# Yash-10/beta-sgp

Measured on AMD Instinct MI355X. Metric: SGP iterations/sec (fp64) on batched 256x256 images, higher is better.
Workload: dtype f64; 1 GPU; C3: 1024 independent 256x256 stamps per GPU, 25x25 PSF, linear A, beta-SGP (beta=1.05), proj_type=1, MAXIT=100, stop_criterion=1; images_per_gpu=1024, images_total=1024, maxit=100, parallelism=1 independent shards, one process per GPU (no collective on the data path), ls_spec=2, streams=1, team=1, proj_cache=1, gn_compact=1, storage=f64, persistent=1, stop_criterion=1

## Files before the change

### beta-sgp_amd/_bsgp.py

```python
import ctypes
import os
import threading

import numpy as np

try:
    import torch
except ImportError:
    torch = None

_HERE = os.path.dirname(os.path.abspath(__file__))
LIB_PATH = os.environ.get("BSGP_LIB", os.path.join(_HERE, "libbsgp.so"))

BSGP_CONV_CIRCULAR = 0
BSGP_CONV_LINEAR_FILL = 1
BSGP_VARIANT_KL = 0
BSGP_VARIANT_BETA = 1
BSGP_STORAGE_F64 = 0
BSGP_STORAGE_F32 = 1
ABI_VERSION = 3
BSGP_ERR_ARG = -1
BSGP_ERR_HIP = -2
BSGP_ERR_UNSUPPORTED = -3
BSGP_ERR_PSF = -4
# ... 595 lines not shown
        raise ValueError(f"storage must be 'f64' or 'f32', not {storage!r}")
    return STORAGE[storage]


_libc = ctypes.CDLL(None)
_libc.memcmp.restype = ctypes.c_int
_libc.memcmp.argtypes = [ctypes.c_void_p, ctypes.c_void_p, ctypes.c_size_t]


def _same_psf(plan, psf):
    ref = plan._psf_host
    return ref.shape == psf.shape and (
        psf.nbytes == 0 or _libc.memcmp(ref.ctypes.data, psf.ctypes.data, psf.nbytes) == 0)


_PLAN_KNOBS = ("BSGP_PERWAVE_MIN_WG", "BSGP_PERWAVE_TW", "BSGP_COOP_ELEMS", "BSGP_LS_PREDICT")


def _plan_key(H, W, psf, conv_mode, storage):
    psf = np.ascontiguousarray(psf, dtype="<f8")
    flat = psf.reshape(-1)
    sample = flat[::max(1, flat.size // 4096)].tobytes()
    return psf, (H, W, psf.shape, hash(sample), conv_mode, storage_code(storage),
                 torch.cuda.current_device(), tuple(os.environ.get(k) for k in _PLAN_KNOBS))


def _new_plan(H, W, psf, key):
    p = Plan(H, W, psf, key[4], key[6], storage=key[5], psf_checked=True)
    p._psf_host = psf.copy()
    return p

# ... 139 lines not shown
```

### beta-sgp_amd/csrc/bsgp_device.hpp

```cpp
#pragma once

#include <hip/hip_runtime.h>
#include <stdint.h>

#include <type_traits>

#include "bsgp_fft.hpp"
#include "bsgp_lanesplit.hpp"
#include "bsgp_math.hpp"
#include "bsgp_reduce.hpp"

namespace bsgp {

constexpr int kTeamFlags = 64;
constexpr int kPartBufs = 3;
constexpr unsigned long long kPartEmpty = 0xFFF75EE0FFF75EE0ull;
constexpr unsigned int kPartEmptyWord = 0xFFF75EE0u;
constexpr int kSharedBytes = 512;

constexpr int kPhaseSlots = 40;
#ifdef BSGP_PHASE_PROF
static __device__ unsigned long long g_phase[kPhaseSlots];
#define PH_T(v) const unsigned long long v = __builtin_amdgcn_s_memtime()
#define PH_ADD(slot, t0)                                                                 \
// ... 48 lines not shown
struct SGeo {
  static constexpr int H = H_, W = W_, P = P_, Q = Q_;
  static constexpr int Qh = Q_ / 2 + 1;
  static constexpr int nfw = kWaves, nfc = kWaves, coop = 0;
  static constexpr int maxlen = P_ > Q_ ? P_ : Q_;
  static constexpr int lpad = (maxlen + 1 > 2 * Qh ? maxlen + 1 : 2 * Qh) | 1;
  static constexpr int sld = H_ + (H_ & 1);
  static constexpr int tw2 = 0, twmix = -1;
  static constexpr int lds_fft_bytes = nfw * 2 * lpad * (int)sizeof(cd);
  static constexpr int lds_tw_p =
      lds_fft_bytes + kWaves * kMaxRed * (int)sizeof(double) + kSharedBytes;
  static constexpr int lds_tw_q = P_ == Q_ ? lds_tw_p : lds_tw_p + P_ * (int)sizeof(cd);
  static constexpr int lds_bytes = lds_tw_q + Q_ * (int)sizeof(cd);
  static constexpr SPlan<P_, lds_tw_p> fp{};
  static constexpr SPlan<Q_, lds_tw_q> fq{};
  const cd* tfA;
  const cd* tfAT;
  size_t tf_stride;
};
template <class GT>
struct IsStaticGeo : std::false_type {};
template <int H_, int W_, int P_, int Q_>
struct IsStaticGeo<SGeo<H_, W_, P_, Q_>> : std::true_type {};
using SGeo256 = SGeo<256, 256, 270, 270>;
static_assert(SGeo256::Qh == 136 && SGeo256::sld == 256 && SGeo256::lpad == 273, "geometry");

template <bool COMP = true, int N, int OFF, class Sync>
__device__ __forceinline__ cd* fft_any(cd* a, cd* b, const SPlan<N, OFF>&, bool inv, int lane,
                                       int nlanes, Sync sync) {
  extern __shared__ __attribute__((aligned(16))) char bsgp_dyn_lds[];
  const cd* t = reinterpret_cast<const cd*>(bsgp_dyn_lds + OFF);
  return fft_run_static<N, COMP>(a, b, t, inv, lane, nlanes, sync);
}

__device__ __forceinline__ void copy_tw(const FftPlan& f) {
  if (f.lds_tw < 0) return;
  extern __shared__ __attribute__((aligned(16))) char bsgp_dyn_lds[];
  cd* d = reinterpret_cast<cd*>(bsgp_dyn_lds + f.lds_tw);
  for (int i = threadIdx.x; i < f.n; i += kBlock) d[i] = f.tw[i];
}
// ... 1284 lines not shown
      A[u] = ldp<NT>(col);
      const cd bk = ldp<NT>(col + (two ? 1 : 0));
      B[u] = two ? bk : cmk(0.0, 0.0);
    }
#pragma unroll
    for (int u = 0; u < kGCH; ++u) {
      const int k = k0 + 64 * u;
      if (k < G.Qh) {
        a[k] = cmk(A[u].x - B[u].y, A[u].y + B[u].x);
        if (k > 0 && G.Q - k >= G.Qh) a[G.Q - k] = cmk(A[u].x + B[u].y, B[u].x - A[u].y);
      }
    }
  }
}

typedef __attribute__((address_space(3))) void lds_void_t;
typedef __attribute__((address_space(1))) void gbl_void_t;
template <unsigned POL = 0, class GT = Geo>
__device__ __forceinline__ void stage_pair(const GT& G, const cd* spec, int ld, int r, bool two,
                                           cd* F, int lane) {
  constexpr int kAux = (POL & kNtSR) ? 2 : 0;
  for (int k0 = 0; k0 < G.Qh; k0 += 32) {
    const int k = k0 + (lane >> 1);
    if (k < G.Qh) {
      const cd* col = spec + (size_t)k * ld + r + (two ? (lane & 1) : 0);
      __builtin_amdgcn_global_load_lds((gbl_void_t*)col, (lds_void_t*)(F + 2 * k0), 16, 0, kAux);
    }
  }
}
template <class GT = Geo>
// ... 133 lines not shown
        }
        in2[j] = cmk(va, vb);
      }
      wave_sync();
      cd* Y = fft_any(in2, Z, G.fq, false, lane, 64, WaveSync());
      for (int k = lane; k < G.Qh; k += 64) {
        cd ak, bk;
        r2c_split(Y, G.Q, k, &ak, &bk);
        store_pair(spec + (size_t)k * G.sld + r, two, pair_ok, ak, bk);
      }
      wave_sync();
    }
  }
}

template <int JCH = kJCH, bool COMP = true, unsigned POL = 0, class LD, class CP, class GT = Geo>
__device__ __forceinline__ void row_inv_fwd2(const GT& G, const Part& D, const cd* src, cd* dst,
                                             cd* lds, LD&& ld, CP&& cp) {
  using V = decltype(ld(0, 0));
  const int w = threadIdx.x >> 6, lane = threadIdx.x & 63;
  const bool pair_ok = (G.sld & 1) == 0;
  if (w < G.nfw) {
    cd* a = lds + w * 2 * G.lpad;
    cd* b = a + G.lpad;
    for (int r = 2 * (D.gw0 + w); r < G.H; r += 2 * D.gws) {
      const bool two = row_two(G, r, G.H);
      gather_pair<POL>(G, src, G.sld, r, two, a, lane);
      V v0[JCH], v1[JCH];
      load_rows<JCH>(ld, r, two, 0, lane, G.W, v0, v1);
      wave_sync();
      cd* Z = fft_any<COMP>(a, b, G.fq, true, lane, 64, WaveSync());
      cd* in2 = (Z == a) ? b : a;
      for (int j0 = 0; j0 < G.Q; j0 += 64 * JCH) {
        if (j0 > 0 && j0 < G.W) load_rows<JCH>(ld, r, two, j0, lane, G.W, v0, v1);
#pragma unroll
        for (int u = 0; u < JCH; ++u) {
          const int j = j0 + 64 * u + lane;
          if (j < G.Q) {
            double va = 0.0, vb = 0.0;
            if (j < G.W) {
              const cd z = Z[j];
              va = cp(r, j, z.x, v0[u]);
              if (two) vb = cp(r + 1, j, z.y, v1[u]);
            }
            in2[j] = cmk(va, vb);
          }
        }
      }
      wave_sync();
      cd* Y = fft_any<COMP>(in2, Z, G.fq, false, lane, 64, WaveSync());
      for (int k = lane; k < G.Qh; k += 64) {
        cd ak, bk;
        r2c_split(Y, G.Q, k, &ak, &bk);
        store_pair<POL>(dst + (size_t)k * G.sld + r, two, pair_ok, ak, bk);
      }
      wave_sync();
    }
  }
}

template <bool COOP = false, unsigned POL = 0, class GT = Geo>
__device__ __forceinline__ void col_conv(const GT& G, const Part& D, cd* spec, const cd* tf,
                                         cd* lds) {
  constexpr bool NT = (POL & kNtSC) != 0;
  if constexpr (COOP) {
    coop_col_conv(G, D, spec, tf, lds);
    return;
  }
  const int w = threadIdx.x >> 6, lane = threadIdx.x & 63;
// ... 353 lines not shown
```

### beta-sgp_amd/csrc/bsgp_internal.hpp

```cpp
#pragma once

#include <hip/hip_runtime.h>

#include <vector>

#include "../../include/bsgp.h"
#include "bsgp_device.hpp"

namespace bsgp {

struct ImgState {
  int par, Xones, stop, iter, epoch;
  int bar_base;
  int64_t E_p, E_ls, ls_passes, status, ls_series;
  int64_t proj_passes, proj_list;
  double sc, flux, bks_scalar, lo, hi, Dcoeff, tol, t0;
  double fv, alpha, tau, lr, init_lr, beta, lam_p, gd, lam;
  double lam_ratio, kappa;
  double konst;
  int g32;
  int par_tf;
  int par_spec;
  double gfill;
  double Valpha[32];
// ... 29 lines not shown
  unsigned int* tctr;
  int* tfail;
  double* plist;
  size_t plist_stride;
  int lcap;
  int list_lds;
  PwProg pw;
  int storage;
  size_t spec_off;
  int ls_cap;
  unsigned spin_limit;
  int fold_setup;
  int ls_predict;
  cd* spec2;
  size_t spec2_stride;
};

hipError_t launch_setup(const SolveArgs& a, size_t lds, hipStream_t s);
hipError_t launch_iteration(const SolveArgs& a, int K, size_t lds, hipStream_t s,
                            hipEvent_t* ev = nullptr);
hipError_t launch_track(const SolveArgs& a, int it, hipStream_t s);
hipError_t launch_build_tf(const Geo& g, const double* kc, cd* spec, cd* tf, double scale,
                           int conj, size_t lds, hipStream_t s);
hipError_t launch_build_tfs(const Geo& g, int n, const double* kc, size_t kc_stride, cd* spec,
                            size_t spec_stride, cd* tf, size_t tf_stride, double scale, int conj,
                            size_t lds, hipStream_t s);
hipError_t launch_place_psfs(const Geo& g, int n, const double* psfs, int kh, int kw, int circ,
                             double* kc, double* sums, hipStream_t s);
hipError_t launch_apply_op(const Geo& g, int B, int transpose, const double* x, double* out,
                           cd* specws, size_t spec_stride, int grid, size_t lds, hipStream_t s);
// ... 5 lines not shown
                             int max_projs, double* x, double* info, hipStream_t s);
hipError_t launch_beta_div(int n, const double* y, const double* x, double beta, double* out,
                           hipStream_t s);
hipError_t launch_beta_div_deriv(int64_t n, const double* y, const double* x, double beta,
                                 double* out, hipStream_t s);
hipError_t launch_grad_parts(int64_t n, const double* den, const double* gn, double beta,
                             double* pow1, double* w, hipStream_t s);
hipError_t set_solver_lds_limit(size_t bytes);
hipError_t team_resident_per_cu(bool coop, int storage, size_t lds, int* per_cu);
hipError_t phase_prof(unsigned long long* out, int n, int reset);
hipError_t launch_persist(const SolveArgs& a, int K, size_t lds, hipStream_t s, unsigned* queue,
                          unsigned* done, int grid);
hipError_t persist_resident_per_cu(const SolveArgs& a, int K, size_t lds, int* per_cu);
bool persist_static_geo(const SolveArgs& a, int K);
bool persist_speculates(const SolveArgs& a);
hipError_t persist_phase_prof(unsigned long long* out, int n, int reset);
void persist_kernels_all(std::vector<const void*>& f);

static_assert(sizeof(bsgp_state_header) <= BSGP_STATE_HEADER_BYTES, "state header overflows");

struct StateLayout {
  size_t bytes, discr, crit, times, flags, x, g, xtf, pw, gn, bkg;
};
inline size_t state_pad16(size_t v) { return (v + 15) / 16 * 16; }
inline StateLayout state_layout(size_t N, int storage, bool bmap, int hist_cap) {
  const size_t vb = storage == BSGP_STORAGE_F32 ? 4 : 8;
  StateLayout L{};
  size_t o = BSGP_STATE_HEADER_BYTES;
  auto take = [&](size_t n) {
    const size_t at = o;
// ... 68 lines not shown
```

### beta-sgp_amd/csrc/bsgp_kernels.hpp

```cpp
#pragma once

#include <hip/hip_runtime.h>

#include <type_traits>
#include <vector>

#include "bsgp_device.hpp"
#include "bsgp_internal.hpp"

namespace bsgp {


#ifndef BSGP_LS1_PRE
#define BSGP_LS1_PRE false
#endif
constexpr int kLs1Jch = 1;
#ifndef BSGP_COL_ATTR
#define BSGP_COL_ATTR
#endif
#ifndef BSGP_LS_ATTR
#define BSGP_LS_ATTR __attribute__((amdgpu_waves_per_eu(COOP ? 1 : ((K <= 2 && !ADAPT) ? 3 : 2))))
#endif
#ifndef BSGP_LS1_K2
#define BSGP_LS1_K2 0
#endif
#ifndef BSGP_PERSIST_LL
#define BSGP_PERSIST_LL 0
#endif
#ifndef BSGP_STREAM_NT
#define BSGP_STREAM_NT 0
#endif
#ifndef BSGP_STATIC_GEO
#define BSGP_STATIC_GEO 0
#endif
constexpr int kLsLanes = 32;
#ifndef BSGP_ACC_SERIES
#define BSGP_ACC_SERIES 0
#endif
constexpr int kLsAccJch = 1;
constexpr bool kLsAccPf = true;
#ifndef BSGP_LS1_PIPE
#define BSGP_LS1_PIPE false
// ... 543 lines not shown
    }
  }
}

template <bool COOP, class V>
__global__ void __launch_bounds__(kBlock) k_setup(SolveArgs A) {
  load_tw_lds(A.g);
  setup_phase<COOP, V>(A, team_img(A));
}

constexpr double kProjGuessW = 0.3;
constexpr double kProjW1 = 0.1;
constexpr double kProjW2 = 0.2;
constexpr int kProjWidePx = 16;

template <class V, bool LL, unsigned POL = 0>
__device__ __forceinline__ ProjOut cached_projection(const SolveArgs& A, int img, const Part& Pt, Team& tm,
                                     const Dir& D, const Bufs<V>& B, double* red, cd* lds,
                                     double lam_prev, double flux, int npair, bool odd, int N,
                                     int64_t& passes, int64_t& list_reads, double lam_ratio,
                                     double kappa, double& first_lam) {
  const V* xa = B.xa;
  const V* ga = B.ga;
  const int LS = tm.T * kBlock;
  const int gt = tm.m * kBlock + (int)threadIdx.x;
  double* ly = A.plist + (size_t)img * A.plist_stride;
  double* lX = ly + A.plist_stride / 2;
  const int lcap = A.lcap;
  const int nl = LL ? A.list_lds : 0;
  double* const qy = reinterpret_cast<double*>(lds);
  double* const qX = qy + (size_t)nl * kBlock;
  const int tl = (int)threadIdx.x;
  const bool hs = D.clip.has_sat;
  const double satv = D.clip.satv;
  bool have = false;
  double cL = 0.0, cU = 0.0, SA = 0.0, SB = 0.0, nsat = 0.0, nstr = 0.0;
  double Lk = -INFINITY, Uk = INFINITY;
  double xl0 = NAN, xs0 = 0.0, xl1 = NAN, xs1 = 0.0, lamN = NAN;
  bool first_miss = true;
  int calls = 0;
  int cnt = 0;

  auto note = [&](double lam, double S) {
    const double r = S - flux;
    if (r < 0 && lam > Lk) Lk = lam;
    if (r > 0 && lam < Uk) Uk = lam;
// ... 19 lines not shown
        t[k] += v;
        if (k == 0 && v > 0.0 && (!hs || v < satv)) t[NL + 5] += X;
      }
      if (split) {
        const double vL = D.pv(y, X, qL), vU = D.pv(y, X, qU);
        if (vU == 0.0) {
        } else if (hs && vL == satv) {
          t[NL + 2] += 1.0;
        } else if (vL > 0.0 && (!hs || vU < satv)) {
          t[NL] += y;
          t[NL + 1] += X;
        } else if (cnt < lcap) {
          if (cnt < nl) {
            qy[cnt * kBlock + tl] = y;
            qX[cnt * kBlock + tl] = X;
          } else {
            ly[(size_t)cnt * LS + gt] = y;
            lX[(size_t)cnt * LS + gt] = X;
          }
          ++cnt;
          t[NL + 3] += 1.0;
        } else {
          t[NL + 4] += 1.0;
        }
      }
    };
    stream2<kProjU>(
        Pt, npair,
        [&](int p) {
          struct Ld {
// ... 19 lines not shown
      SB = t[NL + 1];
      nsat = t[NL + 2];
      nstr = t[NL + 3];
    }
    ++passes;
    PH_ADD(NL == 3 ? 10 : 12, tp0);
    return t[NL + 5];
  };
  auto leval = [&](double lam) {
    PH_T(tl0);
    double t[1] = {0.0};
    int k = 0;
    if (nl > 0) {
      const int kl = cnt < nl ? cnt : nl;
      for (; k < kl; ++k) t[0] += D.pv(qy[k * kBlock + tl], qX[k * kBlock + tl], lam);
    }
    for (; k + 4 <= cnt; k += 4) {
      double yv[4], Xv[4];
#pragma unroll
      for (int u = 0; u < 4; ++u) {
        yv[u] = ly[(size_t)(k + u) * LS + gt];
        Xv[u] = lX[(size_t)(k + u) * LS + gt];
      }
#pragma unroll
      for (int u = 0; u < 4; ++u) t[0] += D.pv(yv[u], Xv[u], lam);
    }
    for (; k < cnt; ++k) t[0] += D.pv(ly[(size_t)k * LS + gt], lX[(size_t)k * LS + gt], lam);
    team_sum<1>(t, red, tm);
    PH_ADD(11, tl0);
    const double lin = SA + lam * SB;
// ... 51 lines not shown
        }
        first_miss = false;
        const double lams[1] = {lam};
        double Sv[1];
        (void)pass(std::integral_constant<int, 1>{}, lams, Sv, split, qL, qU);
        S = Sv[0];
      }
    }
    ++calls;
    note(lam, S);
    return S;
  };
  return project_df_fn(sumf, flux, 0.0, 1.0, 1e-11, 0, 0, A.prm.max_projs);
}

template <bool COOP, class V, bool LL = true, unsigned POL = 0, class GT = Geo>
__device__ __forceinline__ void dir_phase(const SolveArgs& A, int img) {
  constexpr bool kO16 = (POL & kNtO16) != 0, kO8 = (POL & kNtO8) != 0;
  BSGP_LDS_VIEWS_G(A, GT);
  ImgState& st = A.st[img];
  PH_T(tk0);
  Team tm = team_of<GT>(A, img, st);
  decltype(auto) G = geo_of<GT>(A);
  const Part Pt = make_part(tm, G.nfw, G.W);
  const bsgp_params& P = A.prm;
  const int N = G.H * G.W;
  const int npair = (N + 1) / 2;
  const bool odd = (N & 1) != 0;
  Bufs<V> B = slot_bufs<V>(A, img, st.par, st.par_tf);
  Dir D = make_dir(A, st);
  const double flux = st.flux;
// ... 216 lines not shown
      have2 = true;
      PH_ADD(34, tr0);
    }
  };
  bool spec_acc = false;
  bool spec_miss = false;
  if constexpr (kPredBuild) {
    if (pred == 1) {
      double ts[2] = {0.0, 0.0};
      const double bm1s = obj.beta - 1;
      V* const xs = B.xtf2;
      V* const ps = B.pw2;
      struct SpIn {
        double x0, g, bkv;
      };
      row_inv_fwd2<kLs1Jch, kLsComp, POL>(
          G, Pt, B.spec, B.spec2, lds,
          [&](int r, int j) {
            const int i = r * G.W + j;
            SpIn q;
            q.x0 = ldp<kO8>(B.xtf + i);
            q.g = g_raw<kO8>(g32, B.gns, i);
            q.bkv = opt_ld<kO8>(bmap, B.bks, i, bks_scalar);
            return q;
          },
          [&](int r, int j, double v, const SpIn& q) {
            const int i = r * G.W + j;
            const double g = gdec(q.g);
            const double xt = q.x0 + lam * v;
            const double den = xt + q.bkv;
            const double p = fpow(den, bm1s);
            ts[0] += obj.c1 * (den * p);
            ts[1] += (MODE == 4 ? (double)(obj.c2f * (float)g) : obj.c2 * g) * p;
            stp<kW>(xs + i, (V)xt);
            stp<kW>(ps + i, (V)p);
            return g * (p / den);
          });
      team_sum<2>(ts, red, tm);
      PH_ADD(37, tk0);
      ++passes;
      ++nls;
      const double f1 = obj.combine(konst, ts[0], ts[1], flux, (double)N);
      if (f1 <= fr + P.gamma * lam * gd || lam < 1e-12) {
        f_acc = f1;
        accepted = true;
        spec_acc = true;
      } else {
        spec_miss = true;
      }
    }
  }
  if (pred != 1 || spec_miss) {
// ... 521 lines not shown
__device__ __forceinline__ const SolveArgs& args_of(ArgRef r) {
  typedef const __attribute__((address_space(4))) SolveArgs* KP;
  const unsigned lo = (unsigned)__builtin_amdgcn_readfirstlane((int)r.lo);
  const unsigned hi = (unsigned)__builtin_amdgcn_readfirstlane((int)r.hi);
  const unsigned long long a = ((unsigned long long)hi << 32) | (unsigned long long)lo;
  KP p = (KP)a;
  asm volatile("" : "+s"(p));
  return *(const SolveArgs*)p;
}
template <bool COOP, class V>
__device__ __attribute__((noinline)) void persist_setup(ArgRef r, int img) {
  setup_phase<COOP, V>(args_of(r), __builtin_amdgcn_readfirstlane(img));
}
template <bool COOP, class V, unsigned POL, class GT = Geo>
__device__ __attribute__((noinline)) void persist_dir(ArgRef r, int img) {
  dir_phase<COOP, V, (BSGP_PERSIST_LL) != 0, POL, GT>(args_of(r),
                                                    __builtin_amdgcn_readfirstlane(img));
}
template <bool COOP, unsigned POL, class GT = Geo>
__device__ __attribute__((noinline)) void persist_col_a(ArgRef r, int img) {
  const SolveArgs& A = args_of(r);
  img = __builtin_amdgcn_readfirstlane(img);
  BSGP_LDS_VIEWS_G(A, GT);
  (void)red;
  Team tm{};
  tm.T = 1;
  const Bufs<double> Bd = slot_bufs<double>(A, img, 0);
  PH_T(tc0);
  decltype(auto) G = geo_of<GT>(A);
  col_conv<COOP, POL>(G, make_part(tm, COOP ? G.nfc : G.nfw, G.W), Bd.spec, tf_of(G, img, 0), lds);
  PH_ADD(3, tc0);
}
// ... 353 lines not shown
```

### beta-sgp_amd/csrc/bsgp_layout.hpp

```cpp
#pragma once

#include <algorithm>
#include <cerrno>
#include <cstddef>
#include <cstdlib>
#include <string>
#include <vector>

#include "../../include/bsgp.h"
#include "bsgp_fft.hpp"

namespace bsgp {

inline thread_local std::string g_err;

inline int fail(int code, const std::string& msg) {
  g_err = msg;
  return code;
}

inline size_t round_up(size_t v, size_t m) { return (v + m - 1) / m * m; }

inline long long env_knob(const char* name, long long def, long long lo, long long hi) {
  const char* e = getenv(name);
  if (!e || !*e) return def;
  char* end = nullptr;
  errno = 0;
  const long long v = strtoll(e, &end, 10);
  if (errno != 0 || end == e || *end != '\0' || v < lo || v > hi) return def;
  return v;
}

namespace layout {
constexpr int kWaves = 4, kMaxRed = 24, kSharedBytes = 512, kCoopBlock = 512, kCoopGroups = 4;
constexpr size_t kLdsPerCu = 160 * 1024;
}

struct PlanKnobs {
  int perwave_min_wg;
  int perwave_tw;
  int coop_elems;
  static PlanKnobs from_env() {
    return {(int)env_knob("BSGP_PERWAVE_MIN_WG", 2, 2, 4), (int)env_knob("BSGP_PERWAVE_TW", 1, 0, 1),
            (int)env_knob("BSGP_COOP_ELEMS", 8, 4, 8)};
  }
};

struct PlanLayout {
  int H, W, P, Q, Qh, sld, lpad, nfw, nfc, coop, tw2, twmix;
  FftPlan fp, fq;
// ... 47 lines not shown
    if (pmin < km) pmin = km;
    if (qmin < km) qmin = km;
    g.P = next_fast_len(pmin);
    g.Q = next_fast_len(qmin);
  }
  g.Qh = g.Q / 2 + 1;
  g.sld = H + ((H & 1) ? 1 : 0);
  g.fp.n = g.P;
  g.fq.n = g.Q;
  if (!plan_radices(g.P, g.fp.radix, &g.fp.ns) || !plan_radices(g.Q, g.fq.radix, &g.fq.ns))
    return fail(BSGP_ERR_UNSUPPORTED, "FFT length has too many factors");
  const int maxlen = g.P > g.Q ? g.P : g.Q;
  g.lpad = (maxlen + 1 > 2 * g.Qh ? maxlen + 1 : 2 * g.Qh) | 1;
  size_t red_bytes = (size_t)kWaves * kMaxRed * sizeof(double) + kSharedBytes;
  auto need = [&](int n) { return (size_t)n * 2 * g.lpad * sizeof(cd) + red_bytes; };
  auto budget_at = [](int wg) { return kLdsPerCu / wg - 256; };
  size_t budget = budget_at(4);
  g.wg_per_cu = 4;
  const size_t twb = (size_t)(g.P == g.Q ? g.P : g.P + g.Q) * sizeof(cd);
  const size_t tw_need = knobs.perwave_tw ? twb : 0;
  for (int wg = 3; wg >= 2 && wg >= knobs.perwave_min_wg; --wg)
    if (need(kWaves) > budget && need(kWaves) + tw_need <= budget_at(wg)) {
      budget = budget_at(wg);
      g.wg_per_cu = wg;
      break;
    }
  int nfw = kWaves;
  if (need(kWaves) > budget) {
    g.coop = 1;
    budget = budget_at(1);
    red_bytes = (size_t)(kCoopBlock / 64) * kMaxRed * sizeof(double) + kSharedBytes;
// ... 24 lines not shown
  if (g.coop) {
    place_coop_tables(&g);
  } else if (g.lds_bytes + twb <= budget) {
    g.fp.lds_tw = (int)g.lds_bytes;
    g.fq.lds_tw = g.P == g.Q ? g.fp.lds_tw : (int)(g.lds_bytes + (size_t)g.P * sizeof(cd));
    g.lds_bytes += twb;
  }
  g.vec_stride = round_up((size_t)H * W, 32);
  const size_t vbytes = storage == BSGP_STORAGE_F32 ? sizeof(float) : sizeof(double);
  g.spec_off = 2 * g.vec_stride + 7 * g.vec_stride * vbytes / sizeof(double);
  g.slot_stride = g.spec_off + round_up((size_t)g.sld * g.Qh * 2, 32) + 2 * g.vec_stride;
  *out = g;
  return BSGP_OK;
}

inline int check_plan_shape(int H, int W, int kh, int kw, int conv_mode, int storage) {
  if (storage != BSGP_STORAGE_F64 && storage != BSGP_STORAGE_F32)
    return fail(BSGP_ERR_ARG, "bad storage");
  if (H < 1 || W < 1 || kh < 1 || kw < 1) return fail(BSGP_ERR_ARG, "bad shape or psf");
  if (conv_mode != BSGP_CONV_CIRCULAR && conv_mode != BSGP_CONV_LINEAR_FILL)
    return fail(BSGP_ERR_ARG, "bad conv_mode");
  if (conv_mode == BSGP_CONV_CIRCULAR && (kh != H || kw != W))
    return fail(BSGP_ERR_ARG,
                "circular A (use_original_SGP_Afunction=True) needs psf.shape == gn.shape");
  return BSGP_OK;
}

struct PwBuild {
  std::vector<int> leaves, nodes_tmp, heights, roots;
  int rec(int start, int n, int* h) {
// ... 54 lines not shown
```

### beta-sgp_amd/csrc/bsgp_persist.hip

```cpp
#include <hip/hip_runtime.h>

#include <vector>

#ifndef BSGP_LS1_K2
#define BSGP_LS1_K2 1
#endif
#ifndef BSGP_STREAM_NT
#define BSGP_STREAM_NT 21
#endif
#ifndef BSGP_STATIC_GEO
#define BSGP_STATIC_GEO 1
#endif
#ifndef BSGP_PERSIST_LL
#define BSGP_PERSIST_LL 1
#endif
#include "bsgp_kernels.hpp"

namespace bsgp {

hipError_t launch_persist_f32(const SolveArgs& a, int K, size_t lds, hipStream_t s,
                              unsigned* queue, unsigned* done, int grid);
const void* persist_kernel_f32(int K, int mode, bool adapt, bool scalar_bkg);
void persist_kernels_f32(std::vector<const void*>& f);

hipError_t launch_persist(const SolveArgs& a, int K, size_t lds, hipStream_t s, unsigned* queue,
                          unsigned* done, int grid) {
  if (a.g.coop) return bsgp_c512_launch_persist(&a, K, lds, s, queue, done, grid);
  if (app_static_plan(a.g, a.storage))
    return bsgp_app_launch_persist(&a, K, lds, s, queue, done, grid);
// ... 3 lines not shown

bool persist_static_geo(const SolveArgs& a, int K) {
  if (a.g.coop || app_static_plan(a.g, a.storage) || a.storage != BSGP_STORAGE_F64) return false;
  bool adapt = false;
  const int mode = ls_mode(a, &adapt);
  return static_geo_kernel<double, (BSGP_STATIC_GEO != 0)>(false, K >= 2 ? 2 : K, mode, adapt) &&
         static_geo_plan(a);
}

bool persist_speculates(const SolveArgs& a) {
  if (a.g.coop || app_static_plan(a.g, a.storage) || a.storage != BSGP_STORAGE_F64) return false;
  bool adapt = false;
  const int mode = ls_mode(a, &adapt);
  return (BSGP_LS1_K2) != 0 && !adapt && (mode == 3 || mode == 4) && a.prm.ls_series != 0 &&
         a.T == 1 && a.ls_predict != 0;
}

hipError_t persist_resident_per_cu(const SolveArgs& a, int K, size_t lds, int* per_cu) {
  if (a.g.coop) return bsgp_c512_persist_resident(&a, K, lds, per_cu);
  if (app_static_plan(a.g, a.storage)) return bsgp_app_persist_resident(&a, K, lds, per_cu);
  bool adapt = false;
  const int mode = ls_mode(a, &adapt);
  const bool sb = !a.prm.bkg_is_map;
  const void* f = a.storage == BSGP_STORAGE_F32 ? persist_kernel_f32(K, mode, adapt, sb)
                                                : persist_kernel<double>(K, mode, adapt, sb);
  return hipOccupancyMaxActiveBlocksPerMultiprocessor(per_cu, f, kBlock, lds);
}

hipError_t persist_phase_prof_f32(unsigned long long* out, int n, int reset);
hipError_t persist_phase_prof(unsigned long long* out, int n, int reset) {
// ... 31 lines not shown
```

### beta-sgp_amd/csrc/bsgp_plan.hip

```cpp
#include <cmath>
#include <cstdio>
#include <memory>
#include <vector>

#include "bsgp_host.hpp"

using namespace bsgp;

static_assert(layout::kWaves == kWaves && layout::kMaxRed == kMaxRed &&
                  layout::kSharedBytes == kSharedBytes && layout::kCoopBlock == kCoopBlock &&
                  layout::kCoopGroups == kCoopGroups,
              "bsgp_layout.hpp restates the kernels' constants");

namespace {

std::vector<cd> twiddles(int n) {
  std::vector<cd> t(n);
  const long double pi = 3.141592653589793238462643383279502884L;
  for (int k = 0; k < n; ++k) {
    const long double a = -2.0L * pi * (long double)k / (long double)n;
    t[k] = cmk((double)cosl(a), (double)sinl(a));
  }
  return t;
}

void apply_layout(bsgp_plan p, const PlanLayout& l) {
// ... 284 lines not shown
```

### beta-sgp_amd/csrc/bsgp_solve.hip

```cpp
#include <algorithm>
#include <atomic>
#include <cmath>
#include <cstdio>
#include <cstring>
#include <string>
#include <vector>

#include "bsgp_host.hpp"

using namespace bsgp;

namespace {

int check_params(const bsgp_params* q) {
  if (!q) return fail(BSGP_ERR_ARG, "params is NULL");
  if (q->variant != BSGP_VARIANT_KL && q->variant != BSGP_VARIANT_BETA)
    return fail(BSGP_ERR_ARG, "bad variant");
  if (q->MAXIT < 1) return fail(BSGP_ERR_ARG, "MAXIT must be >= 1");
  if (q->M_alpha < 1 || q->M_alpha > 32) return fail(BSGP_ERR_ARG, "M_alpha must be in [1, 32]");
  if (q->M < 1 || q->M > 32) return fail(BSGP_ERR_ARG, "M must be in [1, 32]");
  if (q->ls_spec < 1 || q->ls_spec > 8) return fail(BSGP_ERR_ARG, "ls_spec must be in [1, 8]");
  if (q->init_recon < 0 || q->init_recon > 3) return fail(BSGP_ERR_ARG, "bad init_recon");
  if (q->proj_type != 0 && q->proj_type != 1) return fail(BSGP_ERR_ARG, "bad proj_type");
  if (q->scale_data < 0 || q->scale_data > 2) return fail(BSGP_ERR_ARG, "bad scale_data");
  if (q->flux_f32 && !(q->gn_f32 && q->scale_data != 2))
    return fail(BSGP_ERR_ARG, "flux_f32 needs gn_f32 with scale_data 0 or 1");
  return BSGP_OK;
}

struct SolveKnobs {
  unsigned spin_limit;
  int ls_predict;
  size_t list_lds;
  int static_geo;
  int fold_setup;
  static SolveKnobs from_env() {
    return {(unsigned)env_knob("BSGP_SPIN_LIMIT", 1ll << 26, 0, 0xffffffffll),
            (int)env_knob("BSGP_LS_PREDICT", 1, 0, 5),
            (size_t)env_knob("BSGP_LIST_LDS", 1 << 20, 0, 1 << 20),
            (int)env_knob("BSGP_STATIC_GEO", 1, 0, 1), (int)env_knob("BSGP_FOLD_SETUP", 1, 0, 1)};
  }
};

struct StaticGeoCall {
  bsgp_plan p;
  explicit StaticGeoCall(bsgp_plan q) : p(q) { p->last_static_geo = 0; }
  ~StaticGeoCall() { p->static_geo_next = -1; }
};

int proj_list_cap(const Geo& g, int T) {
  const long npair = ((long)g.H * g.W + 1) / 2;
  const int nb = plan_block(g);
  if (T == 1) return (int)(2 * ((npair + nb - 1) / nb));
  const long cp = (long)g.nfw * g.W;
  const long nch = (npair + cp - 1) / cp;
// ... 29 lines not shown
struct ResumeCtx {
  StateArgs sa;
  int T;
  int it0;
  bool uniform;
  int done_it;
  int beta0_given;
};

struct SolvePath {
  bool data_stop;
  bool track;
  bool persist;
  int K;
  int S;
};

int validate_solve(bsgp_plan p, int32_t B, const bsgp_params* prm, const bsgp_inputs* in,
                   const bsgp_outputs* out, bool resumed) {
  if (!p) return fail(BSGP_ERR_ARG, "plan is NULL");
  if (int rc = check_params(prm)) return rc;
  if (B < 1) return fail(BSGP_ERR_ARG, "B must be >= 1");
  if (!resumed) {
    if (!in || !in->gn || !in->bkg) return fail(BSGP_ERR_ARG, "inputs gn/bkg missing");
    if ((prm->init_recon == 1 || prm->scale_data == 2) && !in->x0)
      return fail(BSGP_ERR_ARG, "init_recon=1 and scale_data=2 need x0");
  }
  if (!out || !out->x || !out->iters || !out->discr) return fail(BSGP_ERR_ARG, "outputs missing");
  if (out->err && (!in || !in->obj)) return fail(BSGP_ERR_ARG, "err needs the ground truth obj");
  if (p->n_tf > 1 && B != p->n_tf)
// ... 39 lines not shown
  a.fuse_col = T == 1 ? 2 : 0;
  a.static_geo = 0;
  a.fold_setup = 0;
  a.tpart = T > 1 ? p->tpart.p : nullptr;
  a.tctr = p->tctr;
  a.tfail = reinterpret_cast<int*>(p->tctr + (size_t)B * kTeamWords);
  a.plist = nullptr;
  a.plist_stride = 0;
  a.lcap = 0;
  a.list_lds = 0;
  a.pw = p->pw;
  a.storage = p->storage;
  a.spec_off = p->spec_off;
  a.spec2 = nullptr;
  a.spec2_stride = 0;
  a.spin_limit = knobs.spin_limit;
  a.ls_predict = knobs.ls_predict;
  a.ls_cap = (prm->beta > 0.0 && prm->beta < 1.0)
                 ? (int)std::ceil(std::log(1e-12) / std::log(prm->beta)) + 2
                 : 4096;
  a.done_host = p->done_d;
  if (prm->proj_cache && prm->proj_type == 1) {
    a.lcap = proj_list_cap(p->g, T);
    const size_t half = round_up((size_t)a.lcap * T * plan_block(p->g), 32);
    a.plist_stride = 2 * half;
    HIP_TRY(p->plist.reserve((size_t)B * a.plist_stride));
    a.plist = p->plist;
    const size_t fit = p->lds_fft_bytes / ((size_t)plan_block(p->g) * 2 * sizeof(double));
    if (T > 1)
      a.list_lds = (int)std::min<size_t>((size_t)a.lcap, fit);
// ... 9 lines not shown
  const bsgp_params& prm = a.prm;
  SolvePath& w = *path;
  w.data_stop = prm.stop_criterion >= 2 && prm.stop_criterion <= 4;
  w.track = a.out.err != nullptr || a.out.x_iter != nullptr;
  w.K = (prm.adapt_beta && prm.variant == BSGP_VARIANT_BETA)
            ? 1
            : (prm.ls_spec <= 1 ? 1 : prm.ls_spec <= 2 ? 2 : prm.ls_spec <= 4 ? 4 : 8);
  w.S = std::min(std::min(std::max(prm.streams, 1), (int)bsgp_plan_s::kMaxStreams), B);
  w.persist = prm.persistent && a.T == 1 && !w.track && (!rs || w.data_stop || rs->uniform);
  if (w.persist) w.S = 1;
  if (w.persist && persist_speculates(a)) {
    HIP_TRY(p->spec2.reserve((size_t)B * spec2_stride(p)));
    a.spec2 = p->spec2;
    a.spec2_stride = spec2_stride(p);
  }
  const int want = p->static_geo_next >= 0 ? p->static_geo_next : knobs.static_geo;
  a.static_geo = (want && w.persist && persist_static_geo(a, w.K)) ? 1 : 0;
  p->last_static_geo = a.static_geo;
  a.fold_setup = (w.persist && !w.data_stop && !rs && knobs.fold_setup) ? 1 : 0;
  return BSGP_OK;
}

int ensure_streams(bsgp_plan p, int S) {
  if (S <= 1 || p->nsub >= S) return BSGP_OK;
  if (!p->ev_fork) HIP_TRY(hipEventCreateWithFlags(&p->ev_fork, hipEventDisableTiming));
  for (int i = (p->nsub > 1 ? p->nsub : 1); i < S; ++i) {
    HIP_TRY(hipStreamCreateWithFlags(&p->sub[i], hipStreamNonBlocking));
    HIP_TRY(hipEventCreateWithFlags(&p->ev_join[i], hipEventDisableTiming));
  }
  p->nsub = S;
// ... 49 lines not shown
    if (!a.fold_setup && !resumed) HIP_TRY(launch_setup(sa[j], p->lds_bytes, ss[j]));
    if (prof) HIP_TRY(hipEventRecord(prof->ev[1], ss[j]));
    if (w.track) HIP_TRY(launch_track(sa[j], 0, ss[j]));
  }
  return BSGP_OK;
}

int run_persistent(bsgp_plan p, const SolveArgs& a, const SolvePath& w, const ResumeCtx* rs,
                   const StateArgs* ld, hipStream_t s, SolveProf* prof) {
  const int B = a.B;
  const size_t need = (size_t)2 * B + 4;
  HIP_TRY(p->pq.reserve(need));
  HIP_TRY(hipMemsetAsync(p->pq, 0, need * sizeof(unsigned), s));
  if (rs && !w.data_stop)
    HIP_TRY(launch_state_post(*ld, B, p->pq, p->pq + 1, rs->done_it, p->done_d, a.seq, s));
  int per_cu = 0;
  HIP_TRY(persist_resident_per_cu(a, w.K, p->lds_bytes, &per_cu));
  if (per_cu < 1) return fail(BSGP_ERR_HIP, "persistent solver does not fit a CU");
  const int grid = (int)std::min<long>(B, (long)p->ncu * per_cu);
  if (prof) HIP_TRY(hipEventRecord(prof->ev[2], s));
  HIP_TRY(launch_persist(a, w.K, p->lds_bytes, s, p->pq, p->pq + 1, grid));
  if (prof) HIP_TRY(hipEventRecord(prof->ev[3], s));
  return BSGP_OK;
}

int run_phased(bsgp_plan p, const SolvePath& w, int it0, int MAXIT, int seq, const hipStream_t* ss,
               const SolveArgs* sa, SolveProf* prof, int* it_run) {
  constexpr int kLook = 2;
  constexpr int kRing = bsgp_plan_s::kPollRing;
  if (w.data_stop)
    for (int i = 0; i < kRing; ++i)
      if (!p->ev_it[i]) HIP_TRY(hipEventCreateWithFlags(&p->ev_it[i], hipEventDisableTiming));
  for (int it = it0; it <= MAXIT; ++it) {
    *it_run = it;
    for (int j = 0; j < w.S; ++j) {
      HIP_TRY(launch_iteration(sa[j], w.K, p->lds_bytes, ss[j],
// ... 392 lines not shown
```

Before: 316,000 image-iterations/s.

## Use spare per-CU LDS for projection lists and staged next-row spectrum prefetch

Computes the LDS left over at the resident workgroup count and hands it to the persistent kernel. By default (LL=2) the projection cache spills list entries into this spare LDS before falling back to global memory. An optional compile-time path prefetches the next row pair's spectrum into spare LDS with async global-to-LDS loads, overlapping the inverse/forward row FFTs. The launch LDS size grows, but only when occupancy stays unchanged. This adds complexity and extra waitcnt synchronization.

```diff
diff --git a/beta-sgp_amd/_bsgp.py b/beta-sgp_amd/_bsgp.py
--- a/beta-sgp_amd/_bsgp.py
+++ b/beta-sgp_amd/_bsgp.py
@@ -633,7 +633,8 @@
         psf.nbytes == 0 or _libc.memcmp(ref.ctypes.data, psf.ctypes.data, psf.nbytes) == 0)
 
 
-_PLAN_KNOBS = ("BSGP_PERWAVE_MIN_WG", "BSGP_PERWAVE_TW", "BSGP_COOP_ELEMS", "BSGP_LS_PREDICT")
+_PLAN_KNOBS = ("BSGP_PERWAVE_MIN_WG", "BSGP_PERWAVE_TW", "BSGP_COOP_ELEMS", "BSGP_LS_PREDICT",
+               "BSGP_FUSED_STAGE")
 
 
 def _plan_key(H, W, psf, conv_mode, storage):
diff --git a/beta-sgp_amd/csrc/bsgp_device.hpp b/beta-sgp_amd/csrc/bsgp_device.hpp
--- a/beta-sgp_amd/csrc/bsgp_device.hpp
+++ b/beta-sgp_amd/csrc/bsgp_device.hpp
@@ -86,6 +86,9 @@
   static constexpr int lds_bytes = lds_tw_q + Q_ * (int)sizeof(cd);
   static constexpr SPlan<P_, lds_tw_p> fp{};
   static constexpr SPlan<Q_, lds_tw_q> fq{};
+  static constexpr int stage_cols_fit =
+      ((160 * 1024 / 3 / 1280 * 1280 - (lds_bytes + 15) / 16 * 16) / 16 * 16 / kWaves / 16 * 16) / 32;
+  static constexpr int stage_cols = stage_cols_fit < Qh ? stage_cols_fit : Qh;
   const cd* tfA;
   const cd* tfAT;
   size_t tf_stride;
@@ -96,6 +99,7 @@
 struct IsStaticGeo<SGeo<H_, W_, P_, Q_>> : std::true_type {};
 using SGeo256 = SGeo<256, 256, 270, 270>;
 static_assert(SGeo256::Qh == 136 && SGeo256::sld == 256 && SGeo256::lpad == 273, "geometry");
+static_assert(kWaves != 4 || SGeo256::stage_cols == 103, "spare LDS at three workgroups per CU");
 
 template <bool COMP = true, int N, int OFF, class Sync>
 __device__ __forceinline__ cd* fft_any(cd* a, cd* b, const SPlan<N, OFF>&, bool inv, int lane,
@@ -1410,6 +1414,7 @@
   }
 }
 
+constexpr int kStageRegCols = 32;
 typedef __attribute__((address_space(3))) void lds_void_t;
 typedef __attribute__((address_space(1))) void gbl_void_t;
 template <unsigned POL = 0, class GT = Geo>
@@ -1573,18 +1578,98 @@
   }
 }
 
-template <int JCH = kJCH, bool COMP = true, unsigned POL = 0, class LD, class CP, class GT = Geo>
+template <int JCH = kJCH, bool COMP = true, unsigned POL = 0, bool STG = false, class LD, class CP,
+          class GT = Geo>
 __device__ __forceinline__ void row_inv_fwd2(const GT& G, const Part& D, const cd* src, cd* dst,
-                                             cd* lds, LD&& ld, CP&& cp) {
+                                             cd* lds, LD&& ld, CP&& cp, cd* stage = nullptr,
+                                             int cs_arg = 0) {
   using V = decltype(ld(0, 0));
   const int w = threadIdx.x >> 6, lane = threadIdx.x & 63;
   const bool pair_ok = (G.sld & 1) == 0;
+  if constexpr (!STG) {
+    if (w < G.nfw) {
+      cd* a = lds + w * 2 * G.lpad;
+      cd* b = a + G.lpad;
+      for (int r = 2 * (D.gw0 + w); r < G.H; r += 2 * D.gws) {
+        const bool two = row_two(G, r, G.H);
+        gather_pair<POL>(G, src, G.sld, r, two, a, lane);
+        V v0[JCH], v1[JCH];
+        load_rows<JCH>(ld, r, two, 0, lane, G.W, v0, v1);
+        wave_sync();
+        cd* Z = fft_any<COMP>(a, b, G.fq, true, lane, 64, WaveSync());
+        cd* in2 = (Z == a) ? b : a;
+        for (int j0 = 0; j0 < G.Q; j0 += 64 * JCH) {
+          if (j0 > 0 && j0 < G.W) load_rows<JCH>(ld, r, two, j0, lane, G.W, v0, v1);
+  #pragma unroll
+          for (int u = 0; u < JCH; ++u) {
+            const int j = j0 + 64 * u + lane;
+            if (j < G.Q) {
+              double va = 0.0, vb = 0.0;
+              if (j < G.W) {
+                const cd z = Z[j];
+                va = cp(r, j, z.x, v0[u]);
+                if (two) vb = cp(r + 1, j, z.y, v1[u]);
+              }
+              in2[j] = cmk(va, vb);
+            }
+          }
+        }
+        wave_sync();
+        cd* Y = fft_any<COMP>(in2, Z, G.fq, false, lane, 64, WaveSync());
+        for (int k = lane; k < G.Qh; k += 64) {
+          cd ak, bk;
+          r2c_split(Y, G.Q, k, &ak, &bk);
+          store_pair<POL>(dst + (size_t)k * G.sld + r, two, pair_ok, ak, bk);
+        }
+        wave_sync();
+      }
+    }
+    return;
+  }
+  bool on = cs_arg > 0;
+  if constexpr (IsStaticGeo<GT>::value) on = on && cs_arg == GT::stage_cols;
   if (w < G.nfw) {
-    cd* a = lds + w * 2 * G.lpad;
-    cd* b = a + G.lpad;
-    for (int r = 2 * (D.gw0 + w); r < G.H; r += 2 * D.gws) {
+    constexpr int kAux = (POL & kNtSR) ? 2 : 0;
+    constexpr bool NT = (POL & kNtSR) != 0;
+    const int cs = [&]() {
+      if constexpr (IsStaticGeo<GT>::value)
+        return (int)GT::stage_cols;
+      else
+        return cs_arg;
+    }();
+    cd* const a = lds + w * 2 * G.lpad;
+    cd* const b = a + G.lpad;
+    cd* const S = stage + (size_t)w * 2 * cs;
+    cd* const T = a + G.Q;
+    const int rest = G.Qh - cs;
+    const bool tailc = rest > kStageRegCols;
+    const int nreg = tailc ? kStageRegCols : rest;
+    auto put = [&](int k, const cd& A, const cd& B) __attribute__((always_inline)) {
+      a[k] = cmk(A.x - B.y, A.y + B.x);
+      if (k > 0 && G.Q - k >= G.Qh) a[G.Q - k] = cmk(A.x + B.y, B.x - A.y);
+    };
+    int r = 2 * (D.gw0 + w);
+    if (r < G.H) gather_pair<POL>(G, src, G.sld, r, row_two(G, r, G.H), a, lane);
+    for (; r < G.H; r += 2 * D.gws) {
       const bool two = row_two(G, r, G.H);
-      gather_pair<POL>(G, src, G.sld, r, two, a, lane);
+      const int rn = r + 2 * D.gws;
+      const bool next = rn < G.H, two_n = row_two(G, rn, G.H);
+      auto nsrc = [&]() __attribute__((always_inline)) {
+        return src + rn + (two_n ? (lane & 1) : 0);
+      };
+      if constexpr (STG) {
+        if (on && next) {
+          for (int k0 = 0; k0 < cs; k0 += 32) {
+            const int k = k0 + (lane >> 1);
+            if (k < cs)
+              __builtin_amdgcn_global_load_lds((gbl_void_t*)(nsrc() + (size_t)k * G.sld),
+                                               (lds_void_t*)(S + 2 * k0), 16, 0, kAux);
+          }
+          if (tailc && lane < 2)
+            __builtin_amdgcn_global_load_lds((gbl_void_t*)(nsrc() + (size_t)(G.Qh - 1) * G.sld),
+                                             (lds_void_t*)T, 16, 0, kAux);
+        }
+      }
       V v0[JCH], v1[JCH];
       load_rows<JCH>(ld, r, two, 0, lane, G.W, v0, v1);
       wave_sync();
@@ -1606,12 +1691,37 @@
           }
         }
       }
+      cd rv = cmk(0.0, 0.0);
+      if constexpr (STG) {
+        if (on && next && nreg > 0)
+          rv = ldp<NT>(nsrc() + (size_t)min(cs + (lane >> 1), G.Qh - 1) * G.sld);
+      }
       wave_sync();
       cd* Y = fft_any<COMP>(in2, Z, G.fq, false, lane, 64, WaveSync());
+      if constexpr (STG) {
+        if (on && next) {
+          asm volatile("s_waitcnt vmcnt(0)" ::: "memory");
+          wave_sync();
+        }
+      }
       for (int k = lane; k < G.Qh; k += 64) {
         cd ak, bk;
         r2c_split(Y, G.Q, k, &ak, &bk);
         store_pair<POL>(dst + (size_t)k * G.sld + r, two, pair_ok, ak, bk);
+      }
+      if (next) {
+        if (STG && on) {
+          const cd zero = cmk(0.0, 0.0);
+          for (int k = lane; k < cs; k += 64) put(k, S[2 * k], two_n ? S[2 * k + 1] : zero);
+          if (nreg > 0) {
+            const cd ov = cmk(__shfl_xor(rv.x, 1, 64), __shfl_xor(rv.y, 1, 64));
+            if ((lane & 1) == 0 && (lane >> 1) < nreg)
+              put(cs + (lane >> 1), rv, two_n ? ov : zero);
+          }
+          if (tailc && lane == 0) put(G.Qh - 1, T[0], two_n ? T[1] : zero);
+        } else {
+          gather_pair<POL>(G, src, G.sld, rn, two_n, a, lane);
+        }
       }
       wave_sync();
     }
diff --git a/beta-sgp_amd/csrc/bsgp_internal.hpp b/beta-sgp_amd/csrc/bsgp_internal.hpp
--- a/beta-sgp_amd/csrc/bsgp_internal.hpp
+++ b/beta-sgp_amd/csrc/bsgp_internal.hpp
@@ -67,6 +67,10 @@
   int ls_predict;
   cd* spec2;
   size_t spec2_stride;
+  int spare_off;
+  int spare_bytes;
+  int list_spare;
+  int stage_cols;
 };
 
 hipError_t launch_setup(const SolveArgs& a, size_t lds, hipStream_t s);
@@ -102,6 +106,8 @@
 hipError_t persist_resident_per_cu(const SolveArgs& a, int K, size_t lds, int* per_cu);
 bool persist_static_geo(const SolveArgs& a, int K);
 bool persist_speculates(const SolveArgs& a);
+int persist_spare_uses(const SolveArgs& a);
+hipError_t persist_static_lds(const SolveArgs& a, int K, size_t* bytes);
 hipError_t persist_phase_prof(unsigned long long* out, int n, int reset);
 void persist_kernels_all(std::vector<const void*>& f);
 
diff --git a/beta-sgp_amd/csrc/bsgp_kernels.hpp b/beta-sgp_amd/csrc/bsgp_kernels.hpp
--- a/beta-sgp_amd/csrc/bsgp_kernels.hpp
+++ b/beta-sgp_amd/csrc/bsgp_kernels.hpp
@@ -26,6 +26,9 @@
 #endif
 #ifndef BSGP_PERSIST_LL
 #define BSGP_PERSIST_LL 0
+#endif
+#ifndef BSGP_FUSED_STAGE
+#define BSGP_FUSED_STAGE 0
 #endif
 #ifndef BSGP_STREAM_NT
 #define BSGP_STREAM_NT 0
@@ -599,7 +602,7 @@
 constexpr double kProjW2 = 0.2;
 constexpr int kProjWidePx = 16;
 
-template <class V, bool LL, unsigned POL = 0>
+template <class V, int LL, unsigned POL = 0>
 __device__ __forceinline__ ProjOut cached_projection(const SolveArgs& A, int img, const Part& Pt, Team& tm,
                                      const Dir& D, const Bufs<V>& B, double* red, cd* lds,
                                      double lam_prev, double flux, int npair, bool odd, int N,
@@ -615,6 +618,10 @@
   const int nl = LL ? A.list_lds : 0;
   double* const qy = reinterpret_cast<double*>(lds);
   double* const qX = qy + (size_t)nl * kBlock;
+  const int ns = LL >= 2 ? A.list_spare : 0;
+  extern __shared__ __attribute__((aligned(16))) char bsgp_dyn_lds[];
+  double* const sy = reinterpret_cast<double*>(bsgp_dyn_lds + (LL >= 2 ? A.spare_off : 0));
+  double* const sX = sy + (size_t)ns * kBlock;
   const int tl = (int)threadIdx.x;
   const bool hs = D.clip.has_sat;
   const double satv = D.clip.satv;
@@ -664,6 +671,9 @@
           if (cnt < nl) {
             qy[cnt * kBlock + tl] = y;
             qX[cnt * kBlock + tl] = X;
+          } else if (LL >= 2 && cnt < nl + ns) {
+            sy[(cnt - nl) * kBlock + tl] = y;
+            sX[(cnt - nl) * kBlock + tl] = X;
           } else {
             ly[(size_t)cnt * LS + gt] = y;
             lX[(size_t)cnt * LS + gt] = X;
@@ -713,6 +723,11 @@
     if (nl > 0) {
       const int kl = cnt < nl ? cnt : nl;
       for (; k < kl; ++k) t[0] += D.pv(qy[k * kBlock + tl], qX[k * kBlock + tl], lam);
+    }
+    if constexpr (LL >= 2) {
+      const int ks = cnt < nl + ns ? cnt : nl + ns;
+      for (; k < ks; ++k)
+        t[0] += D.pv(sy[(k - nl) * kBlock + tl], sX[(k - nl) * kBlock + tl], lam);
     }
     for (; k + 4 <= cnt; k += 4) {
       double yv[4], Xv[4];
@@ -794,7 +809,7 @@
   return project_df_fn(sumf, flux, 0.0, 1.0, 1e-11, 0, 0, A.prm.max_projs);
 }
 
-template <bool COOP, class V, bool LL = true, unsigned POL = 0, class GT = Geo>
+template <bool COOP, class V, int LL = 1, unsigned POL = 0, class GT = Geo>
 __device__ __forceinline__ void dir_phase(const SolveArgs& A, int img) {
   constexpr bool kO16 = (POL & kNtO16) != 0, kO8 = (POL & kNtO8) != 0;
   BSGP_LDS_VIEWS_G(A, GT);
@@ -1041,7 +1056,10 @@
       struct SpIn {
         double x0, g, bkv;
       };
-      row_inv_fwd2<kLs1Jch, kLsComp, POL>(
+      constexpr bool kStage = (BSGP_FUSED_STAGE) != 0;
+      extern __shared__ __attribute__((aligned(16))) char bsgp_dyn_lds[];
+      cd* const stg = reinterpret_cast<cd*>(bsgp_dyn_lds + (kStage ? A.spare_off : 0));
+      row_inv_fwd2<kLs1Jch, kLsComp, POL, kStage>(
           G, Pt, B.spec, B.spec2, lds,
           [&](int r, int j) {
             const int i = r * G.W + j;
@@ -1062,7 +1080,8 @@
             stp<kW>(xs + i, (V)xt);
             stp<kW>(ps + i, (V)p);
             return g * (p / den);
-          });
+          },
+          stg, kStage ? A.stage_cols : 0);
       team_sum<2>(ts, red, tm);
       PH_ADD(37, tk0);
       ++passes;
@@ -1614,8 +1633,8 @@
 }
 template <bool COOP, class V, unsigned POL, class GT = Geo>
 __device__ __attribute__((noinline)) void persist_dir(ArgRef r, int img) {
-  dir_phase<COOP, V, (BSGP_PERSIST_LL) != 0, POL, GT>(args_of(r),
-                                                    __builtin_amdgcn_readfirstlane(img));
+  dir_phase<COOP, V, (BSGP_PERSIST_LL), POL, GT>(args_of(r),
+                                               __builtin_amdgcn_readfirstlane(img));
 }
 template <bool COOP, unsigned POL, class GT = Geo>
 __device__ __attribute__((noinline)) void persist_col_a(ArgRef r, int img) {
diff --git a/beta-sgp_amd/csrc/bsgp_layout.hpp b/beta-sgp_amd/csrc/bsgp_layout.hpp
--- a/beta-sgp_amd/csrc/bsgp_layout.hpp
+++ b/beta-sgp_amd/csrc/bsgp_layout.hpp
@@ -34,6 +34,9 @@
 namespace layout {
 constexpr int kWaves = 4, kMaxRed = 24, kSharedBytes = 512, kCoopBlock = 512, kCoopGroups = 4;
 constexpr size_t kLdsPerCu = 160 * 1024;
+constexpr size_t budget_at(int wg) { return kLdsPerCu / wg - 256; }
+constexpr size_t kLdsGranule = 1280;
+constexpr int kStageRegCols = 32;
 }
 
 struct PlanKnobs {
@@ -111,7 +114,7 @@
   g.lpad = (maxlen + 1 > 2 * g.Qh ? maxlen + 1 : 2 * g.Qh) | 1;
   size_t red_bytes = (size_t)kWaves * kMaxRed * sizeof(double) + kSharedBytes;
   auto need = [&](int n) { return (size_t)n * 2 * g.lpad * sizeof(cd) + red_bytes; };
-  auto budget_at = [](int wg) { return kLdsPerCu / wg - 256; };
+  auto budget_at = [](int wg) { return layout::budget_at(wg); };
   size_t budget = budget_at(4);
   g.wg_per_cu = 4;
   const size_t twb = (size_t)(g.P == g.Q ? g.P : g.P + g.Q) * sizeof(cd);
@@ -166,6 +169,34 @@
   return BSGP_OK;
 }
 
+struct SpareLds {
+  size_t off;
+  size_t bytes;
+  int stage_cols;
+  int list_cols;
+};
+inline SpareLds spare_lds(int coop, size_t lds_bytes, size_t static_lds, int Q, int Qh, int lpad,
+                          int wg, int block) {
+  SpareLds s{round_up(lds_bytes, 16), 0, 0, 0};
+  if (coop || wg < 1 || wg >= 4) return s;
+  size_t top = layout::kLdsPerCu / wg / layout::kLdsGranule * layout::kLdsGranule;
+  if (layout::budget_at(wg) < top) top = layout::budget_at(wg);
+  static_lds = round_up(static_lds, 16);
+  if (top < s.off + static_lds + 16) return s;
+  top -= static_lds;
+  s.bytes = (top - s.off) / 16 * 16;
+  s.list_cols = (int)(s.bytes / ((size_t)block * 2 * sizeof(double)));
+  const size_t per_wave = s.bytes / layout::kWaves / 16 * 16;
+  int cs = (int)std::min<size_t>((size_t)Qh, per_wave / (2 * sizeof(cd)));
+  const int tail = lpad - Q >= 2 ? 1 : 0;
+  if (cs < Qh && cs + layout::kStageRegCols + tail < Qh) cs = 0;
+  s.stage_cols = cs;
+  return s;
+}
+inline SpareLds spare_lds(const PlanLayout& l, int wg, size_t static_lds = 0) {
+  return spare_lds(l.coop, l.lds_bytes, static_lds, l.Q, l.Qh, l.lpad, wg, layout::kWaves * 64);
+}
+
 inline int check_plan_shape(int H, int W, int kh, int kw, int conv_mode, int storage) {
   if (storage != BSGP_STORAGE_F64 && storage != BSGP_STORAGE_F32)
     return fail(BSGP_ERR_ARG, "bad storage");
diff --git a/beta-sgp_amd/csrc/bsgp_persist.hip b/beta-sgp_amd/csrc/bsgp_persist.hip
--- a/beta-sgp_amd/csrc/bsgp_persist.hip
+++ b/beta-sgp_amd/csrc/bsgp_persist.hip
@@ -12,7 +12,10 @@
 #define BSGP_STATIC_GEO 1
 #endif
 #ifndef BSGP_PERSIST_LL
-#define BSGP_PERSIST_LL 1
+#define BSGP_PERSIST_LL 2
+#endif
+#ifndef BSGP_FUSED_STAGE
+#define BSGP_FUSED_STAGE 0
 #endif
 #include "bsgp_kernels.hpp"
 
@@ -46,6 +49,21 @@
   const int mode = ls_mode(a, &adapt);
   return (BSGP_LS1_K2) != 0 && !adapt && (mode == 3 || mode == 4) && a.prm.ls_series != 0 &&
          a.T == 1 && a.ls_predict != 0;
+}
+
+int persist_spare_uses(const SolveArgs& a) {
+  if (a.g.coop || app_static_plan(a.g, a.storage) || a.storage != BSGP_STORAGE_F64) return 0;
+  return ((BSGP_PERSIST_LL) >= 2 ? 1 : 0) | ((BSGP_FUSED_STAGE) != 0 ? 2 : 0);
+}
+
+hipError_t persist_static_lds(const SolveArgs& a, int K, size_t* bytes) {
+  bool adapt = false;
+  const int mode = ls_mode(a, &adapt);
+  hipFuncAttributes attr{};
+  const hipError_t e =
+      hipFuncGetAttributes(&attr, persist_kernel<double>(K, mode, adapt, !a.prm.bkg_is_map));
+  *bytes = attr.sharedSizeBytes;
+  return e;
 }
 
 hipError_t persist_resident_per_cu(const SolveArgs& a, int K, size_t lds, int* per_cu) {
diff --git a/beta-sgp_amd/csrc/bsgp_plan.hip b/beta-sgp_amd/csrc/bsgp_plan.hip
--- a/beta-sgp_amd/csrc/bsgp_plan.hip
+++ b/beta-sgp_amd/csrc/bsgp_plan.hip
@@ -9,7 +9,8 @@
 
 static_assert(layout::kWaves == kWaves && layout::kMaxRed == kMaxRed &&
                   layout::kSharedBytes == kSharedBytes && layout::kCoopBlock == kCoopBlock &&
-                  layout::kCoopGroups == kCoopGroups,
+                  layout::kCoopGroups == kCoopGroups &&
+                  layout::kStageRegCols == kStageRegCols,
               "bsgp_layout.hpp restates the kernels' constants");
 
 namespace {
diff --git a/beta-sgp_amd/csrc/bsgp_solve.hip b/beta-sgp_amd/csrc/bsgp_solve.hip
--- a/beta-sgp_amd/csrc/bsgp_solve.hip
+++ b/beta-sgp_amd/csrc/bsgp_solve.hip
@@ -34,11 +34,13 @@
   size_t list_lds;
   int static_geo;
   int fold_setup;
+  int fused_stage;
   static SolveKnobs from_env() {
     return {(unsigned)env_knob("BSGP_SPIN_LIMIT", 1ll << 26, 0, 0xffffffffll),
             (int)env_knob("BSGP_LS_PREDICT", 1, 0, 5),
             (size_t)env_knob("BSGP_LIST_LDS", 1 << 20, 0, 1 << 20),
-            (int)env_knob("BSGP_STATIC_GEO", 1, 0, 1), (int)env_knob("BSGP_FOLD_SETUP", 1, 0, 1)};
+            (int)env_knob("BSGP_STATIC_GEO", 1, 0, 1), (int)env_knob("BSGP_FOLD_SETUP", 1, 0, 1),
+            (int)env_knob("BSGP_FUSED_STAGE", 1, 0, 1)};
   }
 };
 
@@ -98,6 +100,7 @@
   bool persist;
   int K;
   int S;
+  int per_cu;
 };
 
 int validate_solve(bsgp_plan p, int32_t B, const bsgp_params* prm, const bsgp_inputs* in,
@@ -167,6 +170,7 @@
   a.spec_off = p->spec_off;
   a.spec2 = nullptr;
   a.spec2_stride = 0;
+  a.spare_off = a.spare_bytes = a.list_spare = a.stage_cols = 0;
   a.spin_limit = knobs.spin_limit;
   a.ls_predict = knobs.ls_predict;
   a.ls_cap = (prm->beta > 0.0 && prm->beta < 1.0)
@@ -206,6 +210,34 @@
     a.spec2 = p->spec2;
     a.spec2_stride = spec2_stride(p);
   }
+  w.per_cu = 0;
+  if (w.persist) {
+    HIP_TRY(persist_resident_per_cu(a, w.K, p->lds_bytes, &w.per_cu));
+    const int uses = persist_spare_uses(a);
+    if (uses) {
+      const Geo& g = p->g;
+      size_t static_lds = 0;
+      HIP_TRY(persist_static_lds(a, w.K, &static_lds));
+      const SpareLds sp = spare_lds(g.coop, p->lds_bytes, static_lds, g.Q, g.Qh, g.lpad, w.per_cu,
+                                    plan_block(g));
+      int list_spare = 0;
+      if ((uses & 1) && a.plist != nullptr && a.T == 1 && a.list_lds > 0) {
+        const long cap = (long)std::min<size_t>((size_t)a.lcap, knobs.list_lds);
+        list_spare = (int)std::max<long>(0, std::min<long>(sp.list_cols, cap - a.list_lds));
+      }
+      const int stage =
+          ((uses & 2) && knobs.fused_stage && a.spec2 != nullptr) ? sp.stage_cols : 0;
+      int with = 0;
+      if (sp.bytes && (list_spare || stage))
+        HIP_TRY(persist_resident_per_cu(a, w.K, p->lds_bytes + sp.bytes, &with));
+      if (with == w.per_cu && with > 0) {
+        a.spare_off = (int)sp.off;
+        a.spare_bytes = (int)(sp.off - p->lds_bytes + sp.bytes);
+        a.list_spare = list_spare;
+        a.stage_cols = stage;
+      }
+    }
+  }
   const int want = p->static_geo_next >= 0 ? p->static_geo_next : knobs.static_geo;
   a.static_geo = (want && w.persist && persist_static_geo(a, w.K)) ? 1 : 0;
   p->last_static_geo = a.static_geo;
@@ -285,12 +317,11 @@
   HIP_TRY(hipMemsetAsync(p->pq, 0, need * sizeof(unsigned), s));
   if (rs && !w.data_stop)
     HIP_TRY(launch_state_post(*ld, B, p->pq, p->pq + 1, rs->done_it, p->done_d, a.seq, s));
-  int per_cu = 0;
-  HIP_TRY(persist_resident_per_cu(a, w.K, p->lds_bytes, &per_cu));
+  const int per_cu = w.per_cu;
   if (per_cu < 1) return fail(BSGP_ERR_HIP, "persistent solver does not fit a CU");
   const int grid = (int)std::min<long>(B, (long)p->ncu * per_cu);
   if (prof) HIP_TRY(hipEventRecord(prof->ev[2], s));
-  HIP_TRY(launch_persist(a, w.K, p->lds_bytes, s, p->pq, p->pq + 1, grid));
+  HIP_TRY(launch_persist(a, w.K, p->lds_bytes + (size_t)a.spare_bytes, s, p->pq, p->pq + 1, grid));
   if (prof) HIP_TRY(hipEventRecord(prof->ev[3], s));
   return BSGP_OK;
 }
```

Result: no change. 316,300 image-iterations/s, median of 3 (+0.1%).
